# kidusabe1/Imagined-Speech-Decoding

Measured on AMD Instinct MI355X. Metric: trials/sec end-to-end (filterbank+CNN fwd+bwd), higher is better.
Workload: dtype f32; 1 GPU; cfg2: 64ch x 2s@256Hz EEG, 9-band Butterworth(4) filterbank -> STFT(64/32) log band power -> Conv4Layers(576,32)+Linear(32,5) fwd+bwd, softmax-CE, AdamW; trials_per_gpu=4096, global_batch=4096, parallelism=dp1, streams=one stream

## Files before the change

imagined-speech-decoding_amd/_lib.py:

```python
import ctypes as C
import os

from .build import LIB_PATH

ISD_OK = 0
ISD_ERR_INVALID, ISD_ERR_UNSUPPORTED, ISD_ERR_HIP, ISD_ERR_NO_DEVICE = -1, -2, -3, -4
FB_F32, FB_F64, FB_AUTO, FB_MIXED = 0, 1, 2, 3
BP_MAGNITUDE, BP_POWER, BP_LOGPOWER = 0, 1, 2


class IsdError(RuntimeError):
    def __init__(self, code, msg):
        super().__init__(f"libisd_hip error {code}: {msg}")
        self.code = code


class IsdUnsupported(IsdError):
    pass


_p, _i, _i64, _f = C.c_void_p, C.c_int, C.c_int64, C.c_float
_pi, _pd = C.POINTER(C.c_int), C.POINTER(C.c_double)

SIGNATURES = {
    "isd_abi_version": (_i, []),
    "isd_last_error": (C.c_char_p, []),
    "isd_shader_clock_probe": (_i, [_p, _i, _p]),
    "isd_wall_clock_khz": (_i, []),
    "isd_exact_sum_workspace_bytes": (_i64, []),
    "isd_exact_sum": (_i, [_p, _i64, _p, _p, _p]),
    "isd_device_count": (_i, []),
    "isd_adamw_step": (_i, [_p, _p, _p, _p, _i64, C.c_double, C.c_double, C.c_double, C.c_double, C.c_double, _i64,
                       _p, _p, _p]),
    "isd_adamw_multi_step": (_i, [_i, _p, _p, _p, _p, _p, C.c_double, C.c_double, C.c_double, C.c_double, C.c_double,
                             _i64, _p, _p, _p]),
    "isd_fb_plan_create": (_i, [C.POINTER(_p), _i, _i, _pd, _pd, _i]),
    "isd_fb_plan_destroy": (_i, [_p]),
    "isd_fb_plan_precision": (_i, [_p]),
    "isd_fb_forward": (_i, [_p, _p, _p, _i64, _i64, _i64, _p]),
    "isd_stft_plan_create": (_i, [C.POINTER(_p), _i, _i, _i]),
    "isd_stft_plan_destroy": (_i, [_p]),
    "isd_stft_plan_frames": (_i, [_p]),
    "isd_stft_plan_bins": (_i, [_p]),
    "isd_stft_forward": (_i, [_p, _p, _p, _i64, _p]),
    "isd_stft_bandpower": (_i, [_p, _p, _p, _i64, _i64, _i, _i, _pi, _pi, _i, _f, _p]),
    "isd_features_fused": (_i, [_p, _p, _p, _p, _i64, _i64, _pi, _pi, _i, _f, _p]),
    "isd_features_fused_bf16": (_i, [_p, _p, _p, _p, _i64, _i64, _pi, _pi, _i, _f, _p]),
    "isd_features_fused_last_path": (_i, []),
    "isd_features_backward_workspace_bytes": (_i64, [_p, _p, _i64, _i64, _pi, _pi]),
    "isd_features_backward": (_i, [_p, _p, _p, _p, _p, _p, _i64, _i64, _pi, _pi, _i, _f, _p]),
    "isd_attr_mix": (_i, [_p, _p, _p, _p, _p, _i64, _i64, _i, _i64, _i, _p]),
    "isd_attr_accumulate": (_i, [_p, _p, _p, _p, _p, _i64, _i64, _i, _i64, _i, _f, _p]),
    "isd_fir_plan_create": (_i, [C.POINTER(_p), _i, _pd]),
    "isd_fir_plan_destroy": (_i, [_p]),
    "isd_fir_plan_taps": (_i, [_p]),
    "isd_fir_zero_phase_f32": (_i, [_p, _p, _p, _i64, _i, _p]),
    "isd_fir_zero_phase_f64": (_i, [_p, _p, _p, _i64, _i, _p]),
    "isd_conv4_plan_create": (_i, [C.POINTER(_p), _i, _i, _pi, _pi, _i, _i, _i, _i]),
    "isd_conv4_plan_destroy": (_i, [_p]),
    "isd_conv4_plan_set_activation_dtype": (_i, [_p, _i]),
    "isd_conv4_param_count": (_i64, [_p]),
    "isd_conv4_param_offset": (_i64, [_p, _i, _i]),
    "isd_conv4_windows": (_i, [_p, _i64]),
    "isd_conv4_workspace_bytes": (_i64, [_p, _i64, _i64]),
    "isd_conv4_forward": (_i, [_p, _p, _p, _p, _p, _i64, _i64, _p]),
    "isd_conv4_backward": (_i, [_p, _p, _p, _p, _p, _p, _i64, _i64, _p]),
    "isd_conv4_backward_x": (_i, [_p, _p, _p, _p, _p, _p, _p, _i64, _i64, _p]),
    "isd_linear_forward": (_i, [_p, _p, _p, _p, _p, _i64, _i, _i, _i, _p]),
    "isd_linear_residual_forward": (_i, [_p, _p, _p, _p, _p, _i64, _i, _i, _p]),
    "isd_linear_workspace_bytes": (_i64, [_i64, _i, _i]),
    "isd_embed_forward": (_i, [_p, _p, _p, _p, _i64, _i, _i, _p]),
    "isd_embed_backward": (_i, [_p, _p, _p, _p, _i64, _i, _i, _p]),
    "isd_layernorm_forward": (_i, [_p, _p, _p, _p, _p, _i64, _i, _f, _p]),
    "isd_layernorm_backward": (_i, [_p, _p, _p, _p, _p, _p, _p, _i64, _i, _p]),
    "isd_attention_forward": (_i, [_p, _p, _p, _i64, _i, _i, _i, _f, C.c_uint64, _p]),
    "isd_attention_backward": (_i, [_p, _p, _p, _p, _i64, _i, _i, _i, _f, C.c_uint64, _p]),
    "isd_tail_fused_supported": (_i, [_i, _i, _i, _i, _i, _i]),
    "isd_tail_fused_param_count": (_i64, [_i, _i, _i, _i]),
    "isd_tail_fused_save_floats": (_i64, [_i64, _i, _i, _i]),
    "isd_tail_fused_workspace_floats": (_i64, [_i64, _i, _i, _i, _i, _i]),
    "isd_tail_fused_forward": (_i, [_p, _p, _p, _p, _p, _i64, _i, _i, _i, _i, _i, _i, _i, _f, _f, _f, C.c_uint64, _p,
                                    _p]),
    "isd_tail_fused_backward": (_i, [_p, _p, _p, _p, _p, _p, _p, _i64, _i, _i, _i, _i, _i, _i, _i, _f, _f, _f,
                                     C.c_uint64, _p, _p]),
    "isd_linear_backward": (_i, [_p, _p, _p, _p, _p, _p, _p, _p, _i64, _i, _i, _i, _p]),
    "isd_eegnet_plan_create": (_i, [C.POINTER(_p), _i, _i, _i, _i]),
    "isd_featcnn_supported": (_i, [_p, _i64, _i64, _i]),
    "isd_featcnn_step": (_i, [_p, _p, _p, _p, _p, _p, _i, _p, _p, _p, _p, _p, _p, _i64, _i64, _i, _f, _p]),
    "isd_featcnn_step_bf16": (_i, [_p, _p, _p, _p, _p, _p, _i, _p, _p, _p, _p, _p, _p, _i64, _i64, _i, _f, _p]),
    "isd_paperhead_plan_create": (_i, [C.POINTER(_p), _i, _i, _i]),
    "isd_paperhead_plan_destroy": (_i, [_p]),
    "isd_paperhead_param_count": (_i64, [_p]),
    "isd_paperhead_buffer_count": (_i64, [_p]),
    "isd_paperhead_workspace_bytes": (_i64, [_p, _i64]),
    "isd_paperhead_forward": (_i, [_p, _p, _p, _p, _p, _p, _i64, _i, _f, _f, _p]),
    "isd_paperhead_backward": (_i, [_p, _p, _p, _p, _p, _p, _i64, _p]),
    "isd_paperhead_backward_x": (_i, [_p, _p, _p, _p, _p, _p, _p, _i64, _i, _p]),
    "isd_paperhead_forward_stage": (_i, [_p, _i, _p, _p, _p, _p, _p, _i64, _i, _f, _f, _i, _p]),
    "isd_paperhead_backward_stage": (_i, [_p, _i, _p, _p, _p, _p, _p, _i64, _i, _p]),
    "isd_paperhead_sync_block": (_i, [_p, _i64, _i, _i, C.POINTER(C.c_int64), C.POINTER(C.c_int64)]),
    "isd_paperhead_sync_block_kind": (_i, [_i, _i]),
    "isd_eegnet_sync_block_kind": (_i, [_i, _i]),
    "isd_zone_batch_begin": (_i, []),
    "isd_zone_batch_next": (_i, []),
    "isd_zone_batch_launch": (_i, [_p]),
    "isd_zone_batch_abort": (_i, []),
    "isd_cvblock_plan_create": (_i, [C.POINTER(_p), _i, _i, _i]),
    "isd_cvblock_flat_dim": (_i64, [_p]),
    "isd_eegnet_plan_set_seed_counter": (_i, [_p, _p]),
    "isd_eegnet_plan_set_input_dtype": (_i, [_p, _i]),
    "isd_eegnet_plan_destroy": (_i, [_p]),
    "isd_eegnet_param_count": (_i64, [_p]),
    "isd_eegnet_buffer_count": (_i64, [_p]),
    "isd_eegnet_workspace_bytes": (_i64, [_p, _i64]),
    "isd_eegnet_forward": (_i, [_p, _p, _p, _p, _p, _p, _i64, _i, _f, _f, _f, C.c_uint64, _p]),
    "isd_eegnet_backward": (_i, [_p, _p, _p, _p, _p, _p, _i64, _f, C.c_uint64, _p]),
    "isd_eegnet_backward_x": (_i, [_p, _p, _p, _p, _p, _p, _p, _i64, _i, _f, C.c_uint64, _p]),
    "isd_eegnet_forward_stage": (_i, [_p, _i, _p, _p, _p, _p, _p, _i64, _i, _f, _f, _f, C.c_uint64, _i, _p]),
    "isd_eegnet_backward_stage": (_i, [_p, _i, _p, _p, _p, _p, _p, _i64, _f, C.c_uint64, _i, _p]),
    "isd_eegnet_sync_block": (_i, [_p, _i64, _i, _i, C.POINTER(_i64), C.POINTER(_i64)]),
    "isd_softmax_ce_workspace_bytes": (_i64, [_i64]),
    "isd_softmax_ce": (_i, [_p, _p, _i, _p, _p, _p, _p, _i64, _i, _i, _f, _p, _p]),
}

_lib = None


def lib():
    global _lib
    if _lib is None:
        if not os.path.exists(LIB_PATH):
# ... 28 lines not shown
```

imagined-speech-decoding_amd/csrc/fb.hip:

```cpp
#include "common.h"
#include "stft_plan.h"
#include <math.h>
#include <stdlib.h>
#include <vector>
#include <string.h>
#include <type_traits>
#include <atomic>

namespace isd {

constexpr int kL = 32;
constexpr int kSeg = 16 * kL;
constexpr int kPad = kL + 4;
constexpr int kMaxSec = 8;
constexpr int64_t kMaxRows = 0x7fffffffLL / (8 * 8);

struct FbSec {
  double Mp[4][4];
  double P[4];
  double N16d[4];
  double a1d, a2d;
  double hdq[2][kL / 2];
  float a1f, a2f;
  float N16f[4];
// ... 1132 lines not shown
              const float2 sv = rq[kk * 32 + sl];
              R[kk] += (f2){sv.x, sv.y};
            }
          }
        }
        const float2 wn = tw[(4 * j) & (nblk4 - 1)];
        float acc = 0.f;
#pragma unroll
        for (int bq = 0; bq < KB - 2; ++bq) {
          if (bq < nbin) {
            const f2 lo = R[bq], mid = R[bq + 1], hi = R[bq + 2];
            const float sx = hi.x * wn.x + hi.y * wn.y + lo.x * wn.x - lo.y * wn.y;
            const float sy = hi.y * wn.x - hi.x * wn.y + lo.y * wn.x + lo.x * wn.y;
            const float vx = 0.5f * mid.x + 0.25f * sx, vy = 0.5f * mid.y + 0.25f * sy;
            const float pw = (vx * vx + vy * vy) * scale2;
            acc += mode == ISD_BP_MAGNITUDE ? sqrtf(pw) : pw;
          }
        }
        float r = nbin > 0 ? acc / (float)nbin : 0.f;
        if (mode == ISD_BP_LOGPOWER) r = logf(r + eps);
        if (row_ok && j >= 0 && j < J) store_feat(out, j, r, out16);
      }
      wave_lds_sync();
    }
  }
}

__device__ __forceinline__ void ser_dma16(const void* src_lane, unsigned lds_base) {
  asm volatile("s_mov_b32 m0, %0\n\ts_nop 0\n\tglobal_load_lds_dwordx4 %1, off"
               :: "s"(__builtin_amdgcn_readfirstlane(lds_base)), "v"(src_lane) : "memory", "m0");
}

__device__ __forceinline__ float fma_to(float a, float b, float c) {
  float d;
  asm("v_fma_f32 %0, %1, %2, %3" : "=v"(d) : "s"(a), "v"(b), "v"(c));
  return d;
}
__device__ __forceinline__ void fma_over(double& d, double a, double b, double c) {
  asm("v_fma_f64 %0, %1, %2, %3" : "+v"(d) : "s"(a), "v"(b), "v"(c));
}
__device__ __forceinline__ void fma_over_mid(double& d, double a, double c) {
  asm("v_fma_f64 %0, %1, %0, %2" : "+v"(d) : "s"(a), "v"(c));
}

__device__ __forceinline__ void section_serial_f32(f2 (&v)[kL / 2], const SerSec& sc0, double& c1, double& c2) {
  const SerSec& sc = *later(&sc0);
  const float na1 = -sc.a1, na2 = -sc.a2;
  const float n16[4] = {sc.N16[0], sc.N16[1], sc.N16[2], sc.N16[3]};
  const double m0 = sc.M[0], m1 = sc.M[1], m2 = sc.M[2], m3 = sc.M[3];
  float h0[kL / 2], h1[kL / 2];
#pragma unroll
  for (int j = 0; j < kL / 2; ++j) { h0[j] = sc.hq[0][j]; h1[j] = sc.hq[1][j]; }
  const float one = sc.one;
  const f2 NA1 = {na1, na1}, NA2 = {na2, na2}, ONE = {one, one};
  f2 S1 = {0.f, 0.f}, S2 = {0.f, 0.f};
#pragma unroll
  for (int j = 0; j < kL / 2; ++j) {
    const f2 x = v[j];
    const f2 y = j == 0 ? x : __builtin_elementwise_fma(ONE, x, S1);
    S1 = j == 0 ? NA1 * y : __builtin_elementwise_fma(NA1, y, S2);
    S2 = __builtin_elementwise_fma(NA2, y, -x);
    v[j] = y;
  }
  const float sA1 = S1.x, sA2 = S2.x;
  const double e1 = (double)fmaf(n16[0], S1.x, fmaf(n16[1], S2.x, S1.y));
  const double e2 = (double)fmaf(n16[2], S1.x, fmaf(n16[3], S2.x, S2.y));
  const float t1 = (float)c1, t2 = (float)c2;
  const double i1 = fma(m1, c2, e1), i2 = fma(m3, c2, e2);
  fma_over(c2, m2, c1, i2);
  fma_over_mid(c1, m0, i1);
  const float u1 = fma_to(n16[0], t1, fmaf(n16[1], t2, sA1));
  const float u2 = fma_to(n16[2], t1, fmaf(n16[3], t2, sA2));
  const f2 T1 = {t1, u1}, T2 = {t2, u2};
#pragma unroll
  for (int j = 0; j < kL / 2; ++j)
    v[j] = __builtin_elementwise_fma((f2){h0[j], h0[j]}, T1, __builtin_elementwise_fma((f2){h1[j], h1[j]}, T2, v[j]));
}

constexpr int kSerRows = 64;
constexpr int kSerBins = 4;
constexpr int kSerMaxGroups = 4;

constexpr int kSerMaxWaves = 12;
template <int BPW, bool MAG>
__global__ __launch_bounds__(64 * kSerMaxWaves) __attribute__((amdgpu_waves_per_eu(BPW == 1 ? 5 : BPW == 2 ? 4 : 3)))
void fused_serial_kernel(const SerSec* __restrict__ secs, const FbBand* __restrict__ bands,
                         const float2* __restrict__ sym, const float* __restrict__ x, float* __restrict__ feat,
                         int R, int C, int T, int nb, int J, float scale2, FusedBands fbnd, int mode, float eps,
                         const int* __restrict__ bmap, int nb_out, int out16, int NW) {
  constexpr int NS = 4;
  extern __shared__ __attribute__((aligned(16))) float ring_raw[];
  const int lane = threadIdx.x & 63;
  const int wave_all = __builtin_amdgcn_readfirstlane((int)(threadIdx.x >> 6));
  const int grp = wave_all / NW, wave = wave_all - grp * NW;
  float* const ring = ring_raw + grp * (2 * kSerRows * kL);
  const int row0 = (blockIdx.x * (int)(blockDim.x >> 6) / NW + grp) * kSerRows;
  const int row = row0 + lane;
  const bool row_ok = row < R;
  const int rowc = row_ok ? row : R - 1;
  const int bt = rowc / C, ch = rowc - bt * C;
  unsigned obyte = (unsigned)(((int64_t)bt * nb_out * C + ch) * (int64_t)J) << (out16 ? 1 : 2);
  asm volatile("" : "+v"(obyte));
  const int64_t bstride = (int64_t)C * J;
  const int n_chunks = T / kL;

  const unsigned ring_base = (unsigned)(uintptr_t)(__attribute__((address_space(3))) float*)ring;
  auto fetch_tile = [&](int c) {
    if (c >= n_chunks) return;
    for (int i = wave; i < 8; i += NW) {
      const int r = 8 * i + (lane >> 3);
      int gr = row0 + r;
      gr = gr < R ? gr : R - 1;
      const float* src = x + (int64_t)gr * T + c * kL + 4 * ((lane & 7) ^ ((r >> 1) & 7));
      ser_dma16(src, ring_base + (unsigned)(((c & 1) * kSerRows * kL) * 4 + i * 1024));
    }
  };
  const int rbase = lane * kL, rswz = (lane >> 1) & 7;

  double S[BPW][NS][2];
  f2 prevU[BPW][kSerBins];
  float ob[BPW][4];
#pragma unroll
  for (int i = 0; i < BPW; ++i) {
    ob[i][0] = ob[i][1] = ob[i][2] = ob[i][3] = 0.f;
#pragma unroll
    for (int s = 0; s < NS; ++s) S[i][s][0] = S[i][s][1] = 0.0;
#pragma unroll
    for (int kk = 0; kk < kSerBins; ++kk) prevU[i][kk] = (f2){0.f, 0.f};
  }

  int pend = 0;
  fetch_tile(0);
  for (int c = 0; c <= n_chunks; ++c) {
    const bool last = c == n_chunks;
    const float* tile = ring + (c & 1) * (kSerRows * kL);
    if (pend == 1) __builtin_amdgcn_s_waitcnt(0x0F71);
    else if (pend == 2) __builtin_amdgcn_s_waitcnt(0x0F72);
    else if (pend == 3) __builtin_amdgcn_s_waitcnt(0x0F73);
    else __builtin_amdgcn_s_waitcnt(0x0F70);
    __builtin_amdgcn_s_barrier();
    asm volatile("" ::: "memory");
    fetch_tile(c + 1);
    pend = 0;
#pragma unroll
    for (int i = 0; i < BPW; ++i) {
      const int b = wave + i * NW;
      if (b < nb) {
        const int klo = fbnd.klo[b], khi = fbnd.khi[b];
        const int k0 = klo - 1, nbin = khi - klo + 1;
        f2 Xs[kSerBins];
        if (!last) {
          f2 v[kL / 2];
          {
            const float gain = bands[b].gf;
#pragma unroll
            for (int qd = 0; qd < 4; ++qd) {
              const float4 a = *reinterpret_cast<const float4*>(&tile[rbase + ((qd ^ rswz) << 2)]);
              const float4 h = *reinterpret_cast<const float4*>(&tile[rbase + (((qd + 4) ^ rswz) << 2)]);
#pragma unroll
              for (int e = 0; e < 4; ++e)
                v[4 * qd + e] = (f2){mul_unpacked(f4_get(a, e), gain), mul_unpacked(f4_get(h, e), gain)};
            }
          }
#pragma unroll
          for (int s = 0; s < NS; ++s) section_serial_f32(v, secs[b * NS + s], S[i][s][0], S[i][s][1]);
          f2 ad[15];
#pragma unroll
          for (int m = 1; m < 16; ++m) ad[m - 1] = sym_pair(v[m], v[16 - m]);
#pragma unroll
          for (int kk = 0; kk < kSerBins; ++kk) {
            const int k = k0 + kk;
            const f2* __restrict__ tq = later(reinterpret_cast<const f2*>(sym + (int64_t)k * 16));
            f2 tc[17];
#pragma unroll
            for (int m = 1; m <= 16; ++m) tc[m] = tq[m - 1];
            f2 acc_a = pmac0(ad[0], tc[1]), acc_b = pmac0(ad[1], tc[2]);
#pragma unroll
            for (int m = 3; m <= 13; m += 2) {
              pmac(acc_a, ad[m - 1], tc[m]);
              pmac(acc_b, ad[m], tc[m + 1]);
            }
            pmac(acc_a, ad[14], tc[15]);
            cmac_lo_conj(acc_b, v[0], tc[16]);
            f2 U = acc_a + acc_b;
            add_lo(U, v[0]);
            const float sg = __builtin_bit_cast(float, 0x3f800000u | ((unsigned)k << 31));
            Xs[kk] = __builtin_elementwise_fma(U, (f2){sg, sg}, prevU[i][kk]);
            prevU[i][kk] = U;
          }
        } else {
#pragma unroll
          for (int kk = 0; kk < kSerBins; ++kk) Xs[kk] = prevU[i][kk];
        }
        float acc = 0.f;
#pragma unroll
        for (int bq = 0; bq < kSerBins - 2; ++bq) {
          const f2 w = Xs[bq] - Xs[bq + 2], mid = Xs[bq + 1];
          const float vx = fmaf(0.25f, w.y, 0.5f * mid.x), vy = fmaf(-0.25f, w.x, 0.5f * mid.y);
          float pw = (vx * vx + vy * vy) * scale2;
          if (MAG) pw = sqrtf(pw);
          acc += bq < nbin ? pw : 0.f;
        }
        float r = acc * fbnd.inv[b];
        if (mode == ISD_BP_LOGPOWER) r = fast_log(r + eps);
        const int cq = c & 3;
        if (cq == 0) ob[i][0] = r; else if (cq == 1) ob[i][1] = r; else if (cq == 2) ob[i][2] = r; else ob[i][3] = r;
        if ((cq == 3 || last) && row0 < R) pend += (cq == 3) ? 1 : cq + 1;
        if (row_ok && (cq == 3 || last)) {
          const int64_t ou = (int64_t)bmap[b] * bstride + (c - cq);
          if (out16) {
            char* fu = reinterpret_cast<char*>(reinterpret_cast<unsigned short*>(feat) + ou) + obyte;
            if (cq == 3) {
              unsigned p0, p1;
              asm("v_cvt_pk_bf16_f32 %0, %1, %2" : "=v"(p0) : "v"(ob[i][0]), "v"(ob[i][1]));
              asm("v_cvt_pk_bf16_f32 %0, %1, %2" : "=v"(p1) : "v"(ob[i][2]), "v"(ob[i][3]));
              typedef unsigned u2h __attribute__((ext_vector_type(2), aligned(2)));
              *reinterpret_cast<u2h*>(fu) = (u2h){p0, p1};
            } else {
#pragma unroll
              for (int k = 0; k < 3; ++k)
                if (k <= cq) {
                  unsigned pk;
                  asm("v_cvt_pk_bf16_f32 %0, %1, %1" : "=v"(pk) : "v"(ob[i][k]));
                  reinterpret_cast<unsigned short*>(fu)[k] = (unsigned short)pk;
                }
            }
          } else {
            char* fu = reinterpret_cast<char*>(feat + ou) + obyte;
            if (cq == 3) {
              typedef float f4u __attribute__((ext_vector_type(4), aligned(4)));
              *reinterpret_cast<f4u*>(fu) = (f4u){ob[i][0], ob[i][1], ob[i][2], ob[i][3]};
            } else {
#pragma unroll
              for (int k = 0; k < 3; ++k)
                if (k <= cq) reinterpret_cast<float*>(fu)[k] = ob[i][k];
            }
          }
        }
      }
    }
  }
}

static void mat2_mul(const double* a, const double* b, double* o) {
  double r[4] = {a[0] * b[0] + a[1] * b[2], a[0] * b[1] + a[1] * b[3], a[2] * b[0] + a[3] * b[2],
                 a[2] * b[1] + a[3] * b[3]};
  memcpy(o, r, sizeof(r));
}

}

using namespace isd;

extern "C" int isd_fb_plan_destroy(isd_fb_plan* p);

static int rows4_share(int nb) {
  int best = kLongShare;
  double best_w = 1e30;
  for (int s = kLongShare; s >= 4; --s) {
    const int per = (nb + s - 1) / s;
    if (per > kRows4Bands) continue;
    const double w = (double)per * s / (double)(nb > 0 ? nb : 1);
    if (w < best_w - 1e-9) { best_w = w; best = s; }
  }
  return best;
}

static bool rows4_enabled() {
  static const bool on = getenv("ISD_FUSED_ROWS4_OFF") == nullptr;
  return on;
}

static bool rows4_reg_carry() {
  static const bool on = getenv("ISD_ROWS4_LDS_CARRY") == nullptr;
  return on;
}

static void build_section(double a1, double a2, FbSec& sc, double* Qout) {
  const double A[4] = {-a1, 1.0, -a2, 0.0};
  double An[4] = {1, 0, 0, 1};
  for (int k = 0; k < kL; ++k) {
    if (k < kL / 2) {
      sc.hdq[0][k] = An[0];
      sc.hdq[1][k] = An[1];
      sc.hq[0][k] = (float)An[0];
      sc.hq[1][k] = (float)An[1];
    }
    if (k == kL / 2)
      for (int e = 0; e < 4; ++e) {
        sc.N16d[e] = An[e];
        sc.N16f[e] = (float)An[e];
      }
    mat2_mul(A, An, An);
  }
  double Mk[4];
  memcpy(Mk, An, sizeof(Mk));
  double Qi[4] = {1, 0, 0, 1};
  for (int i = 0; i < 16; ++i) {
    memcpy(Qout + i * 4, Qi, sizeof(Qi));
    mat2_mul(Mk, Qi, Qi);
  }
  memcpy(sc.P, Qi, sizeof(Qi));
  for (int k = 0; k < 4; ++k) {
    memcpy(sc.Mp[k], Mk, sizeof(Mk));
    mat2_mul(Mk, Mk, Mk);
  }
  sc.a1d = a1; sc.a2d = a2; sc.a1f = (float)a1; sc.a2f = (float)a2;
}

extern "C" int isd_fb_plan_create(isd_fb_plan** out, int n_bands, int n_sections, const double* a12,
                                  const double* gain, int precision) {
  ISD_CHECK_ARG(out && a12 && gain, "isd_fb_plan_create: null argument");
  ISD_CHECK_ARG(n_bands >= 1 && n_bands <= 4096, "isd_fb_plan_create: n_bands=%d out of range", n_bands);
  ISD_CHECK_ARG(n_sections >= 1 && n_sections <= kMaxSec, "isd_fb_plan_create: n_sections=%d not in [1,%d]",
                n_sections, kMaxSec);
  ISD_CHECK_ARG(precision == ISD_FB_F32 || precision == ISD_FB_F64 || precision == ISD_FB_AUTO,
                "isd_fb_plan_create: bad precision %d", precision);
  const int n = n_bands * n_sections;
  std::vector<FbSec> secs(n);
  std::vector<FbBand> bands(n_bands);
  std::vector<double> Q((size_t)n * 64);
  std::vector<double> worst(n_bands, 0.0);
  for (int b = 0; b < n_bands; ++b) {
    bands[b].gd = gain[b];
// ... 92 lines not shown
    FbSet& fs = p->set[k];
    if (fs.d_sec) (void)hipFree(fs.d_sec);
    if (fs.d_band) (void)hipFree(fs.d_band);
    if (fs.d_Q) (void)hipFree(fs.d_Q);
    if (fs.d_map) (void)hipFree(fs.d_map);
    if (fs.d_ser) (void)hipFree(fs.d_ser);
    delete[] p->host_map[k];
  }
  delete p;
  return ISD_OK;
}

extern "C" int isd_fb_plan_precision(const isd_fb_plan* p) { return p ? p->precision : ISD_ERR_INVALID; }

template <typename VT, int GPR>
static int fb_launch(const isd_fb_plan* p, const FbSet& fs, const float* x, float* y, int64_t R, int C, int T,
                     hipStream_t st) {
  const int64_t items = cdiv(R, (int64_t)(4 / GPR));
  const int vec = ((T & 3) == 0) && ((reinterpret_cast<uintptr_t>(x) & 15) == 0) &&
                  ((reinterpret_cast<uintptr_t>(y) & 15) == 0);
  if (vec && T == GPR * kSeg && R % (4 / GPR) == 0)
    hipLaunchKernelGGL((fb_kernel<VT, GPR, true>), dim3((unsigned)items), dim3(64), 0, st, fs.d_sec, fs.d_band, fs.d_Q, x,
                       y, (int)R, C, T, fs.nb, p->n_sections, vec, fs.d_map, p->n_bands);
  else
    hipLaunchKernelGGL((fb_kernel<VT, GPR>), dim3((unsigned)items), dim3(64), 0, st, fs.d_sec, fs.d_band, fs.d_Q, x, y,
                       (int)R, C, T, fs.nb, p->n_sections, vec, fs.d_map, p->n_bands);
  ISD_LAUNCH_CHECK();
  return ISD_OK;
}

template <typename VT>
static int fb_launch_t(const isd_fb_plan* p, const FbSet& fs, const float* x, float* y, int64_t R, int C, int T,
                       hipStream_t st) {
  if (T <= kSeg) return fb_launch<VT, 1>(p, fs, x, y, R, C, T, st);
  if (T <= 2 * kSeg) return fb_launch<VT, 2>(p, fs, x, y, R, C, T, st);
  const int vec = ((T & 3) == 0) && ((reinterpret_cast<uintptr_t>(x) & 15) == 0) &&
                  ((reinterpret_cast<uintptr_t>(y) & 15) == 0);
  if (vec && T % kSeg == 0 && fs.nb <= kMaxBands && rows4_enabled()) {
    const int share_n = rows4_share(fs.nb);
    const dim3 grid4((unsigned)(cdiv(cdiv(R, 4), 8) * 8 * share_n));
#define ISD_R4(K) hipLaunchKernelGGL(K, grid4, dim3(64), 0, st, fs.d_sec, fs.d_band, fs.d_Q, x, y, C, T, fs.nb, \
                                     p->n_sections, fs.d_map, p->n_bands, (int)R, share_n)
    const bool fullq = R % 4 == 0;
    if (std::is_same<VT, float>::value) { if (fullq) ISD_R4(fb_rows4_kernel_f32<true>); else ISD_R4(fb_rows4_kernel_f32<false>); }
    else { if (fullq) ISD_R4(fb_rows4_kernel_f64<true>); else ISD_R4(fb_rows4_kernel_f64<false>); }
#undef ISD_R4
    ISD_LAUNCH_CHECK();
    return ISD_OK;
  }
  const dim3 grid((unsigned)(cdiv(R, 8) * 8 * kLongShare));
#define ISD_FBL(K) hipLaunchKernelGGL(K, grid, dim3(64), 0, st, fs.d_sec, fs.d_band, fs.d_Q, x, y, C, T, fs.nb, \
                                      p->n_sections, fs.d_map, p->n_bands, (int)R)
  if (std::is_same<VT, float>::value) { if (vec) ISD_FBL(fb_long_kernel_f32<true>); else ISD_FBL(fb_long_kernel_f32<false>); }
  else { if (vec) ISD_FBL(fb_long_kernel_f64<true>); else ISD_FBL(fb_long_kernel_f64<false>); }
#undef ISD_FBL
  ISD_LAUNCH_CHECK();
  return ISD_OK;
}

extern "C" int isd_fb_forward(const isd_fb_plan* p, const float* x, float* y, int64_t B, int64_t C, int64_t T,
                              void* stream) {
  ISD_CHECK_ARG(p, "isd_fb_forward: null plan");
  ISD_CHECK_ARG(B >= 0 && C >= 1 && T >= 1 && T <= (1 << 24) && C <= (1 << 20), "isd_fb_forward: bad shape B=%lld C=%lld T=%lld",
                (long long)B, (long long)C, (long long)T);
  if (B == 0) return ISD_OK;
  ISD_CHECK_ARG(x && y, "isd_fb_forward: null argument");
  hipStream_t st = (hipStream_t)stream;
  const int64_t R = B * C;
  ISD_CHECK_ARG(R <= kMaxRows, "isd_fb_forward: too many rows (%lld)", (long long)R);
  int rc = ISD_OK;
  if (p->set[0].nb) rc = fb_launch_t<float>(p, p->set[0], x, y, R, (int)C, (int)T, st);
  if (rc == ISD_OK && p->set[1].nb) rc = fb_launch_t<double>(p, p->set[1], x, y, R, (int)C, (int)T, st);
  return rc;
}

static void set_band(FusedBands& f, int i, int klo, int khi) {
  f.klo[i] = klo;
  f.khi[i] = khi;
  f.inv[i] = khi >= klo ? 1.f / (float)(khi - klo + 1) : 0.f;
}

static thread_local int g_fused_path = 0;
extern "C" int isd_features_fused_last_path(void) { return g_fused_path; }

static bool serial_wanted() {
  const char* e = getenv("ISD_FUSED_SERIAL");
  return !(e && e[0] == '0');
}

static void serial_lds_limit() {
  static std::atomic<unsigned long long> done{0};
  int dev = 0;
  if (hipGetDevice(&dev) != hipSuccess || dev < 0 || dev >= 64) dev = 0;
  const unsigned long long bit = 1ull << dev;
  if (done.load(std::memory_order_relaxed) & bit) return;
  const int lds = (int)(sizeof(float) * kSerMaxGroups * 2 * kSerRows * kL);
  const void* k[] = {(const void*)fused_serial_kernel<1, false>, (const void*)fused_serial_kernel<1, true>,
                     (const void*)fused_serial_kernel<2, false>, (const void*)fused_serial_kernel<2, true>,
                     (const void*)fused_serial_kernel<3, false>, (const void*)fused_serial_kernel<3, true>};
  for (const void* f : k) (void)hipFuncSetAttribute(f, hipFuncAttributeMaxDynamicSharedMemorySize, lds);
  done.fetch_or(bit, std::memory_order_relaxed);
}

static bool fused_serial_launch(const isd_fb_plan* fb, const FbSet& fs, const isd_stft_plan* st, const float* x,
                                float* feat, int64_t R, int C, const FusedBands& fbnd, int mode, float eps,
                                hipStream_t stream, int out16) {
  if (!serial_wanted() || !st->d_sym || !fs.d_ser || st->n != 64 || st->hop != 32 || st->T % kL != 0 || st->T < kL) return false;
  if (st->J != st->T / kL + 1 || fb->n_sections != 4 || (reinterpret_cast<uintptr_t>(x) & 15) != 0) return false;
  if (fs.nb < 1 || fs.nb > 12) return false;
  if (cdiv(R, C) * (int64_t)fb->n_bands * C * st->J * 4 >= (1LL << 31)) return false;
  for (int i = 0; i < fs.nb; ++i) {
    const int nbin = fbnd.khi[i] - fbnd.klo[i] + 1;
    if (nbin < 1 || nbin > kSerBins - 2 || fbnd.klo[i] < 1 || fbnd.khi[i] > st->n / 2 - 1) return false;
  }
  int bpw = 3;
  if (const char* e = getenv("ISD_SERIAL_BPW")) { const int v = atoi(e); if (v >= 1 && v <= 3) bpw = v; }
  while (bpw < 3 && (fs.nb + bpw - 1) / bpw > kSerMaxWaves) ++bpw;
  const int nw = (fs.nb + bpw - 1) / bpw;
  bpw = (fs.nb + nw - 1) / nw;
  int groups = nw % 4 == 0 ? 1 : nw % 2 == 0 ? 2 : 4;
  while (groups > 1 && groups * nw > kSerMaxWaves) groups >>= 1;
  if (const char* e = getenv("ISD_SERIAL_GROUPS")) { const int v = atoi(e); if (v >= 1 && v <= kSerMaxGroups && v * nw <= kSerMaxWaves) groups = v; }
  const dim3 grid((unsigned)cdiv(R, (int64_t)kSerRows * groups));
  const size_t lds = sizeof(float) * (size_t)groups * 2 * kSerRows * kL;
  const bool mag = mode == ISD_BP_MAGNITUDE;
  if (lds > 48 * 1024) serial_lds_limit();
#define ISD_SER(BPW_)                                                                                                   \
  do {                                                                                                                  \
    if (mag)                                                                                                            \
      hipLaunchKernelGGL((fused_serial_kernel<BPW_, true>), grid, dim3(64 * nw * groups), lds, stream, fs.d_ser,        \
                         fs.d_band, st->d_sym, x, feat, (int)R, C, st->T, fs.nb, st->J, st->scale * st->scale, fbnd,    \
                         mode, eps, fs.d_map, fb->n_bands, out16, nw);                                                  \
    else                                                                                                                \
      hipLaunchKernelGGL((fused_serial_kernel<BPW_, false>), grid, dim3(64 * nw * groups), lds, stream, fs.d_ser,       \
                         fs.d_band, st->d_sym, x, feat, (int)R, C, st->T, fs.nb, st->J, st->scale * st->scale, fbnd,    \
                         mode, eps, fs.d_map, fb->n_bands, out16, nw);                                                  \
  } while (0)
  if (bpw == 1) ISD_SER(1);
  else if (bpw == 2) ISD_SER(2);
  else ISD_SER(3);
#undef ISD_SER
  return true;
}

template <typename VT>
static int fused_launch(const isd_fb_plan* fb, const FbSet& fs, const isd_stft_plan* st, const float* x, float* feat,
                        int64_t R, int C, const FusedBands& fbnd, int mode, float eps, hipStream_t stream, int out16) {
  if (std::is_same<VT, float>::value &&
      fused_serial_launch(fb, fs, st, x, feat, R, C, fbnd, mode, eps, stream, out16)) {
    g_fused_path = 2;
    ISD_LAUNCH_CHECK();
    return ISD_OK;
  }
  if (std::is_same<VT, float>::value) g_fused_path = 1;
  const bool two = st->T > kSeg;
  const int64_t items = cdiv(R, two ? 2 : 4);
  const int vec = ((st->T & 3) == 0) && ((reinterpret_cast<uintptr_t>(x) & 15) == 0);
  const int gpr = two ? 2 : 1;
  const bool full = vec && st->T == gpr * kSeg && R % (4 / gpr) == 0;
#define ISD_FUSED3(M, G, F)                                                                                          \
  hipLaunchKernelGGL((fused_kernel<VT, M, G, F>), dim3((unsigned)items), dim3(64), 0, stream, fs.d_sec, fs.d_band,   \
                     fs.d_Q, st->d_dft, x, feat, (int)R, C, st->T, fs.nb, fb->n_sections, st->J,                     \
                     st->scale * st->scale, fbnd, mode, eps, vec, fs.d_map, fb->n_bands, out16)
#define ISD_FUSED(M, G) do { if (full) ISD_FUSED3(M, G, true); else ISD_FUSED3(M, G, false); } while (0)
  if (mode == ISD_BP_MAGNITUDE) { if (two) ISD_FUSED(true, 2); else ISD_FUSED(true, 1); }
  else { if (two) ISD_FUSED(false, 2); else ISD_FUSED(false, 1); }
#undef ISD_FUSED3
#undef ISD_FUSED
  ISD_LAUNCH_CHECK();
  return ISD_OK;
}

static int features_fused_impl(const isd_fb_plan* fb, const isd_stft_plan* st, const float* x, float* feat,
                               int64_t B, int64_t C, const int* klo, const int* khi, int mode, float eps,
                               void* stream, int out16) {
  ISD_CHECK_ARG(fb && st, "isd_features_fused: null plan");
  ISD_CHECK_ARG(B == 0 || (x && feat), "isd_features_fused: null argument");
  ISD_CHECK_ARG(B >= 0 && C >= 1 && C <= (1 << 20), "isd_features_fused: bad shape B=%lld C=%lld", (long long)B,
                (long long)C);
  ISD_CHECK_ARG(mode >= ISD_BP_MAGNITUDE && mode <= ISD_BP_LOGPOWER, "isd_features_fused: bad mode %d", mode);
  const bool short_rows = st->n == 64 && st->hop == 32 && st->T <= 2 * kSeg && st->d_dft;
  const bool long_rows = st->d_blk && st->hop == 64 && st->T <= 64 * 64;
  if (!short_rows && !long_rows) {
    set_error("isd_features_fused: needs nperseg=64/noverlap=32/T<=1024, or hop 64 with nperseg = 2^a*64 and T<=4096 "
              "(got nperseg=%d hop=%d T=%d)", st->n, st->hop, st->T);
    return ISD_ERR_UNSUPPORTED;
  }
  FusedBands all = {};
  int rc = fill_band_args(st, fb->n_bands, klo, khi, all.klo, all.khi, "isd_features_fused");
  if (rc) return rc;
  if (B == 0) return ISD_OK;
  ISD_CHECK_ARG(B * C <= kMaxRows, "isd_features_fused: too many rows (%lld)", (long long)(B * C));
  hipStream_t s = (hipStream_t)stream;
  if (!short_rows) {
    g_fused_path = 3;
    int nbmax = 0;
    for (int b = 0; b < fb->n_bands; ++b) {
      const int nbin = all.khi[b] - all.klo[b] + 1;
      if (nbin < 1 || nbin > 6 || all.klo[b] < 1 || all.khi[b] > st->n / 2 - 1) {
        set_error("isd_features_fused: band %d needs 1..6 interior bins for the block-sum path (bins %d..%d)", b,
                  all.klo[b], all.khi[b]);
        return ISD_ERR_UNSUPPORTED;
      }
      if (nbin > nbmax) nbmax = nbin;
    }
    const int64_t rows = B * C;
    int log2_nblk = 0;
    while ((64 << log2_nblk) < st->n) ++log2_nblk;
    const int KB = nbmax + 2 <= 4 ? 4 : nbmax + 2 <= 5 ? 5 : nbmax + 2 <= 6 ? 6 : 8;
    const int n_iter = (st->T + 4 * kSeg - 1) / (4 * kSeg);
    const int vec = ((st->T & 3) == 0) && ((reinterpret_cast<uintptr_t>(x) & 15) == 0);
    for (int k = 0; k < 2; ++k) {
      const FbSet& fs = fb->set[k];
      if (!fs.nb) continue;
      FusedBands fbnd = {};
      for (int i = 0; i < fs.nb; ++i) set_band(fbnd, i, all.klo[fb->host_map[k][i]], all.khi[fb->host_map[k][i]]);
      const size_t lds = sizeof(float2) * ((size_t)KB * 64 + 64) + sizeof(double) * (2 * kMaxSec + 64 * kMaxSec);
#define ISD_FL_LAUNCH2(VT, K, V)                                                                                      \
  hipLaunchKernelGGL((fused_long_kernel<VT, K, V>), dim3((unsigned)(cdiv(rows, 8) * 8 * kLongShare)), dim3(64), lds, s, \
                     fs.d_sec, fs.d_band, fs.d_Q, st->d_blk, x, feat, (int)C, st->T, fs.nb, fb->n_sections, st->J,      \
                     log2_nblk, st->n / 2, st->scale * st->scale, fbnd, mode, eps, fs.d_map, fb->n_bands, (int)rows, \
                     out16)
      const bool rows4 = vec && st->T % kSeg == 0 && log2_nblk <= 4 && log2_nblk >= 1 && rows4_enabled();
// ... 355 lines not shown
```

include/isd_hip.h:

```cpp
#ifndef ISD_HIP_H
#define ISD_HIP_H

#include <stdint.h>

#ifdef __cplusplus
extern "C" {
#endif

#define ISD_ABI_VERSION 1

enum {
  ISD_OK = 0,
  ISD_ERR_INVALID = -1,
  ISD_ERR_UNSUPPORTED = -2,
  ISD_ERR_HIP = -3,
  ISD_ERR_NO_DEVICE = -4
};

int isd_abi_version(void);
const char* isd_last_error(void);
int isd_shader_clock_probe(uint64_t* out, int spin_us, void* stream);
int isd_wall_clock_khz(void);
int64_t isd_exact_sum_workspace_bytes(void);
int isd_exact_sum(const float* x, int64_t n, double* out, void* workspace, void* stream);
int isd_device_count(void);

typedef struct isd_fb_plan isd_fb_plan;

enum { ISD_FB_F32 = 0, ISD_FB_F64 = 1, ISD_FB_AUTO = 2, ISD_FB_MIXED = 3  };

int isd_fb_plan_create(isd_fb_plan** out, int n_bands, int n_sections,
                       const double* a12, const double* gain, int precision);
int isd_fb_plan_destroy(isd_fb_plan* plan);
int isd_fb_plan_precision(const isd_fb_plan* plan);

int isd_fb_forward(const isd_fb_plan* plan, const float* x, float* y,
                   int64_t B, int64_t C, int64_t T, void* stream);

typedef struct isd_stft_plan isd_stft_plan;

int isd_stft_plan_create(isd_stft_plan** out, int T, int nperseg, int noverlap);
int isd_stft_plan_destroy(isd_stft_plan* plan);
int isd_stft_plan_frames(const isd_stft_plan* plan);
int isd_stft_plan_bins(const isd_stft_plan* plan);

int isd_stft_forward(const isd_stft_plan* plan, const float* x, float* Z,
                     int64_t R, void* stream);

enum {
  ISD_BP_MAGNITUDE = 0,
  ISD_BP_POWER = 1,
  ISD_BP_LOGPOWER = 2
};

int isd_stft_bandpower(const isd_stft_plan* plan, const float* y, float* feat,
                       int64_t B, int64_t C, int n_bands_in, int n_bands,
                       const int* klo, const int* khi, int mode, float eps, void* stream);

int isd_features_fused(const isd_fb_plan* fb, const isd_stft_plan* st, const float* x,
                       float* feat, int64_t B, int64_t C, const int* klo, const int* khi,
                       int mode, float eps, void* stream);
int isd_features_fused_bf16(const isd_fb_plan* fb, const isd_stft_plan* st, const float* x, uint16_t* feat,
                            int64_t B, int64_t C, const int* klo, const int* khi, int mode, float eps, void* stream);

int isd_features_fused_last_path(void);

int64_t isd_features_backward_workspace_bytes(const isd_fb_plan* fb, const isd_stft_plan* st, int64_t B, int64_t C,
                                              const int* klo, const int* khi);
int isd_features_backward(const isd_fb_plan* fb, const isd_stft_plan* st, const float* x, const float* dfeat,
                          float* dx, void* workspace, int64_t B, int64_t C, const int* klo, const int* khi,
                          int mode, float eps, void* stream);

int isd_attr_mix(const float* x, const float* bg, const int32_t* ridx, const float* alpha, float* out,
                 int64_t n_pairs, int64_t pair0, int S, int64_t E, int M, void* stream);
int isd_attr_accumulate(const float* x, const float* bg, const int32_t* ridx, const float* grad, float* acc,
                        int64_t n_pairs, int64_t pair0, int S, int64_t E, int M, float scale, void* stream);

typedef struct isd_fir_plan isd_fir_plan;
int isd_fir_plan_create(isd_fir_plan** out, int n_taps, const double* taps);
int isd_fir_plan_destroy(isd_fir_plan* plan);
int isd_fir_plan_taps(const isd_fir_plan* plan);
int isd_fir_zero_phase_f32(const isd_fir_plan* plan, const float* x, float* y, int64_t rows, int T, void* stream);
int isd_fir_zero_phase_f64(const isd_fir_plan* plan, const double* x, double* y, int64_t rows, int T, void* stream);

typedef struct isd_conv4_plan isd_conv4_plan;

int isd_conv4_plan_create(isd_conv4_plan** out, int c_total, int n_zones, const int* zone_sizes,
                          const int* zone_channels, int feature_dim, int n_layers, int window_len,
                          int slide_step);
int isd_conv4_plan_destroy(isd_conv4_plan* plan);
enum { ISD_ACT_F32 = 0, ISD_ACT_BF16 = 1 };
int isd_conv4_plan_set_activation_dtype(isd_conv4_plan* plan, int dtype);
int64_t isd_conv4_param_count(const isd_conv4_plan* plan);
int64_t isd_conv4_param_offset(const isd_conv4_plan* plan, int zone, int which);
int isd_conv4_windows(const isd_conv4_plan* plan, int64_t T);
int64_t isd_conv4_workspace_bytes(const isd_conv4_plan* plan, int64_t B, int64_t T);

int isd_conv4_forward(const isd_conv4_plan* plan, const float* x, const float* params, float* feat,
                      void* workspace, int64_t B, int64_t T, void* stream);
int isd_conv4_backward(const isd_conv4_plan* plan, const float* x, const float* params,
                       const float* dfeat, float* dparams, void* workspace, int64_t B, int64_t T,
                       void* stream);
int isd_conv4_backward_x(const isd_conv4_plan* plan, const float* x, const float* params, const float* dfeat,
                         float* dparams, float* dx, void* workspace, int64_t B, int64_t T, void* stream);

int isd_linear_forward(const float* x, const float* w, const float* bias, float* y, float* pre,
                       int64_t M, int K, int N, int act, void* stream);
int isd_linear_residual_forward(const float* x, const float* w, const float* bias, const float* res, float* y,
                                int64_t M, int K, int N, void* stream);
int64_t isd_linear_workspace_bytes(int64_t M, int K, int N);
int isd_linear_backward(const float* x, const float* w, const float* dy, const float* pre, float* dx,
                        float* dw, float* db, void* workspace, int64_t M, int K, int N, int act,
                        void* stream);

int64_t isd_softmax_ce_workspace_bytes(int64_t B);
int isd_softmax_ce(const float* logits_tok, const void* labels, int label_bytes, float* logits_mean,
                   float* loss, float* dlogits_tok, int64_t* pred, int64_t B, int n_tok, int n_cls,
                   float grad_scale, void* workspace, void* stream);

typedef struct isd_eegnet_plan isd_eegnet_plan;
int isd_eegnet_plan_create(isd_eegnet_plan** out, int in_channels, int feature_dim, int kernel_length, int T);
int isd_cvblock_plan_create(isd_eegnet_plan** out, int in_channels, int dim_token, int T);
int64_t isd_cvblock_flat_dim(const isd_eegnet_plan* plan);
int isd_eegnet_plan_set_seed_counter(isd_eegnet_plan* plan, const uint64_t* seed_dev);
int isd_eegnet_plan_set_input_dtype(isd_eegnet_plan* plan, int dtype);
int isd_eegnet_plan_destroy(isd_eegnet_plan* plan);
int64_t isd_eegnet_param_count(const isd_eegnet_plan* plan);
int64_t isd_eegnet_buffer_count(const isd_eegnet_plan* plan);
int64_t isd_eegnet_workspace_bytes(const isd_eegnet_plan* plan, int64_t B);
int isd_eegnet_forward(const isd_eegnet_plan* plan, const float* x, const float* params, float* buffers,
                       float* out, void* workspace, int64_t B, int training, float momentum, float eps,
                       float dropout_p, uint64_t seed, void* stream);
int isd_eegnet_backward(const isd_eegnet_plan* plan, const float* x, const float* params, const float* dout,
                        float* dparams, void* workspace, int64_t B, float dropout_p, uint64_t seed,
                        void* stream);
int isd_eegnet_backward_x(const isd_eegnet_plan* plan, const float* x, const float* params, const float* dout,
                          float* dparams, float* dx, void* workspace, int64_t B, int training, float dropout_p,
                          uint64_t seed, void* stream);
int isd_eegnet_forward_stage(const isd_eegnet_plan* plan, int stage, const float* x, const float* params,
                             float* buffers, float* out, void* workspace, int64_t B, int training, float momentum,
                             float eps, float dropout_p, uint64_t seed, int world, void* stream);
int isd_eegnet_backward_stage(const isd_eegnet_plan* plan, int stage, const float* x, const float* params,
                              const float* dout, float* dparams, void* workspace, int64_t B, float dropout_p,
                              uint64_t seed, int world, void* stream);
int isd_eegnet_sync_block(const isd_eegnet_plan* plan, int64_t B, int backward, int stage, int64_t* byte_offset,
                          int64_t* n_doubles);
int isd_eegnet_sync_block_kind(int backward, int stage);

// ... 74 lines not shown
```

Before: 3.809 million trials/s.

## Stage fused-serial filterbank features in LDS and flush coalesced per frame piece

Adds a staged variant of the fused serial filterbank+STFT kernel. It writes per-row band-power outputs into an LDS staging buffer and flushes them in frame chunks, with lanes spread across rows and frames, instead of each lane scattering 4-frame groups directly to global memory. It also raises the dynamic LDS limit to the full CU size so a staging buffer fits, and sizes the chunk from the occupancy budget. The cost is extra LDS use, which may reduce occupancy, plus extra wave syncs around the flushes.

After: 3.801 million trials/s. No clear change (-0.2%).

```diff
diff --git a/imagined-speech-decoding_amd/_lib.py b/imagined-speech-decoding_amd/_lib.py
--- a/imagined-speech-decoding_amd/_lib.py
+++ b/imagined-speech-decoding_amd/_lib.py
@@ -47,6 +47,7 @@
     "isd_features_fused": (_i, [_p, _p, _p, _p, _i64, _i64, _pi, _pi, _i, _f, _p]),
     "isd_features_fused_bf16": (_i, [_p, _p, _p, _p, _i64, _i64, _pi, _pi, _i, _f, _p]),
     "isd_features_fused_last_path": (_i, []),
+    "isd_features_fused_last_stage": (_i, []),
     "isd_features_backward_workspace_bytes": (_i64, [_p, _p, _i64, _i64, _pi, _pi]),
     "isd_features_backward": (_i, [_p, _p, _p, _p, _p, _p, _i64, _i64, _pi, _pi, _i, _f, _p]),
     "isd_attr_mix": (_i, [_p, _p, _p, _p, _p, _i64, _i64, _i, _i64, _i, _p]),
diff --git a/imagined-speech-decoding_amd/csrc/fb.hip b/imagined-speech-decoding_amd/csrc/fb.hip
--- a/imagined-speech-decoding_amd/csrc/fb.hip
+++ b/imagined-speech-decoding_amd/csrc/fb.hip
@@ -1238,12 +1238,12 @@
 constexpr int kSerMaxGroups = 4;
 
 constexpr int kSerMaxWaves = 12;
-template <int BPW, bool MAG>
+template <int BPW, bool MAG, bool STG>
 __global__ __launch_bounds__(64 * kSerMaxWaves) __attribute__((amdgpu_waves_per_eu(BPW == 1 ? 5 : BPW == 2 ? 4 : 3)))
 void fused_serial_kernel(const SerSec* __restrict__ secs, const FbBand* __restrict__ bands,
                          const float2* __restrict__ sym, const float* __restrict__ x, float* __restrict__ feat,
                          int R, int C, int T, int nb, int J, float scale2, FusedBands fbnd, int mode, float eps,
-                         const int* __restrict__ bmap, int nb_out, int out16, int NW) {
+                         const int* __restrict__ bmap, int nb_out, int out16, int NW, int FS) {
   constexpr int NS = 4;
   extern __shared__ __attribute__((aligned(16))) float ring_raw[];
   const int lane = threadIdx.x & 63;
@@ -1273,6 +1273,55 @@
   };
   const int rbase = lane * kL, rswz = (lane >> 1) & 7;
 
+  const int SS = FS | 1;
+  const int n_pieces = STG ? (J + FS - 1) / FS : 1;
+  float* const stg = ring_raw + (int)(blockDim.x >> 6) / NW * (2 * kSerRows * kL) + wave_all * (BPW * kSerRows * SS + kSerRows);
+  unsigned* const otab = reinterpret_cast<unsigned*>(stg + BPW * kSerRows * SS);
+  float* const stg_lane = stg + lane * SS;
+  if (STG) otab[lane] = row_ok ? obyte : ~0u;
+  auto flush = [&](int f0, int L) {
+    wave_lds_sync();
+    const int q = kSerRows / L, rm = kSerRows - q * L;
+    const int fr0 = lane / L, ff0 = lane - fr0 * L;
+#pragma unroll
+    for (int i = 0; i < BPW; ++i) {
+      const int b = wave + i * NW;
+      if (b < nb) {
+        const int64_t ou = (int64_t)bmap[b] * bstride + f0;
+        char* const fu = out16 ? reinterpret_cast<char*>(reinterpret_cast<unsigned short*>(feat) + ou)
+                               : reinterpret_cast<char*>(feat + ou);
+        int fr = fr0, ff = ff0;
+        for (int k0 = 0; k0 < L; k0 += 4) {
+          float rv[4];
+          unsigned ro[4], fo[4];
+#pragma unroll
+          for (int u = 0; u < 4; ++u) {
+            const int frc = fr < kSerRows ? fr : kSerRows - 1;
+            rv[u] = stg[(i * kSerRows + frc) * SS + ff];
+            ro[u] = otab[frc];
+            fo[u] = (unsigned)ff;
+            fr += q; ff += rm;
+            if (ff >= L) { ff -= L; ++fr; }
+          }
+#pragma unroll
+          for (int u = 0; u < 4; ++u) {
+            if (k0 + u < L && ro[u] != ~0u) {
+              if (out16) {
+                unsigned pk;
+                asm("v_cvt_pk_bf16_f32 %0, %1, %1" : "=v"(pk) : "v"(rv[u]));
+                *reinterpret_cast<unsigned short*>(fu + (ro[u] + 2u * fo[u])) = (unsigned short)pk;
+              } else {
+                *reinterpret_cast<float*>(fu + (ro[u] + 4u * fo[u])) = rv[u];
+              }
+            }
+          }
+        }
+      }
+    }
+  };
+  int pc_lo = 0, pc_hi = J / n_pieces, pc_i = 0;
+  int fl_lo = 0, fl_n = 0;
+
   double S[BPW][NS][2];
   f2 prevU[BPW][kSerBins];
   float ob[BPW][4];
@@ -1296,6 +1345,7 @@
     else __builtin_amdgcn_s_waitcnt(0x0F70);
     __builtin_amdgcn_s_barrier();
     asm volatile("" ::: "memory");
+    if (STG && fl_n) { flush(fl_lo, fl_n); fl_n = 0; }
     fetch_tile(c + 1);
     pend = 0;
 #pragma unroll
@@ -1359,6 +1409,10 @@
         }
         float r = acc * fbnd.inv[b];
         if (mode == ISD_BP_LOGPOWER) r = fast_log(r + eps);
+        if (STG) {
+          stg_lane[i * kSerRows * SS + (c - pc_lo)] = r;
+          continue;
+        }
         const int cq = c & 3;
         if (cq == 0) ob[i][0] = r; else if (cq == 1) ob[i][1] = r; else if (cq == 2) ob[i][2] = r; else ob[i][3] = r;
         if ((cq == 3 || last) && row0 < R) pend += (cq == 3) ? 1 : cq + 1;
@@ -1395,7 +1449,13 @@
         }
       }
     }
-  }
+    if (STG && c + 1 == pc_hi) {
+      fl_lo = pc_lo; fl_n = pc_hi - pc_lo;
+      pc_lo = pc_hi; ++pc_i;
+      pc_hi = (pc_i + 1) * J / n_pieces;
+    }
+  }
+  if (STG && fl_n) flush(fl_lo, fl_n);
 }
 
 static void mat2_mul(const double* a, const double* b, double* o) {
@@ -1654,24 +1714,53 @@
 
 static thread_local int g_fused_path = 0;
 extern "C" int isd_features_fused_last_path(void) { return g_fused_path; }
+static thread_local int g_fused_stage = 0;
+extern "C" int isd_features_fused_last_stage(void) { return g_fused_stage; }
 
 static bool serial_wanted() {
   const char* e = getenv("ISD_FUSED_SERIAL");
   return !(e && e[0] == '0');
 }
 
-static void serial_lds_limit() {
-  static std::atomic<unsigned long long> done{0};
+constexpr int kSerLdsCU = 160 * 1024;
+static int serial_lds_limit() {
+  static std::atomic<unsigned long long> done{0}, wide{0};
   int dev = 0;
   if (hipGetDevice(&dev) != hipSuccess || dev < 0 || dev >= 64) dev = 0;
   const unsigned long long bit = 1ull << dev;
-  if (done.load(std::memory_order_relaxed) & bit) return;
-  const int lds = (int)(sizeof(float) * kSerMaxGroups * 2 * kSerRows * kL);
-  const void* k[] = {(const void*)fused_serial_kernel<1, false>, (const void*)fused_serial_kernel<1, true>,
-                     (const void*)fused_serial_kernel<2, false>, (const void*)fused_serial_kernel<2, true>,
-                     (const void*)fused_serial_kernel<3, false>, (const void*)fused_serial_kernel<3, true>};
-  for (const void* f : k) (void)hipFuncSetAttribute(f, hipFuncAttributeMaxDynamicSharedMemorySize, lds);
-  done.fetch_or(bit, std::memory_order_relaxed);
+  const int tiles = (int)(sizeof(float) * kSerMaxGroups * 2 * kSerRows * kL);
+  if (done.load(std::memory_order_acquire) & bit) return (wide.load(std::memory_order_relaxed) & bit) ? kSerLdsCU : tiles;
+#define ISD_SER_K(B_) (const void*)fused_serial_kernel<B_, false, false>, (const void*)fused_serial_kernel<B_, true, false>, \
+                      (const void*)fused_serial_kernel<B_, false, true>, (const void*)fused_serial_kernel<B_, true, true>
+  const void* k[] = {ISD_SER_K(1), ISD_SER_K(2), ISD_SER_K(3)};
+#undef ISD_SER_K
+  bool ok = true;
+  for (const void* f : k) ok = hipFuncSetAttribute(f, hipFuncAttributeMaxDynamicSharedMemorySize, kSerLdsCU) == hipSuccess && ok;
+  if (!ok) {
+    (void)hipGetLastError();
+    for (const void* f : k) (void)hipFuncSetAttribute(f, hipFuncAttributeMaxDynamicSharedMemorySize, tiles);
+  } else {
+    wide.fetch_or(bit, std::memory_order_relaxed);
+  }
+  done.fetch_or(bit, std::memory_order_release);
+  return ok ? kSerLdsCU : tiles;
+}
+
+static int serial_stage_frames(int J, int bpw, int waves, size_t tile_bytes, int lds_limit) {
+  const char* e = getenv("ISD_SERIAL_STAGE");
+  const int forced = e ? atoi(e) : -1;
+  if (forced == 0) return 0;
+  const int cap = bpw == 1 ? 5 : bpw == 2 ? 4 : 3;
+  const int resident = std::max(1, cap / ((waves + 3) / 4));
+  const int64_t budget = std::min<int64_t>(kSerLdsCU / resident / 2048 * 2048, lds_limit) - (int64_t)tile_bytes;
+  const int64_t ss_max = (budget / waves / 4 - kSerRows) / (bpw * kSerRows);
+  if (budget <= 0 || ss_max < 1) return 0;
+  int fs = (int)std::min<int64_t>(J, ss_max % 2 ? ss_max : ss_max - 1);
+  if (forced > 0) fs = std::min(fs, forced);
+  if (fs < 1) return 0;
+  if (fs < J && fs < 4 && forced <= 0) return 0;
+  const int pieces = (J + fs - 1) / fs;
+  return (J + pieces - 1) / pieces;
 }
 
 static bool fused_serial_launch(const isd_fb_plan* fb, const FbSet& fs, const isd_stft_plan* st, const float* x,
@@ -1694,23 +1783,24 @@
   while (groups > 1 && groups * nw > kSerMaxWaves) groups >>= 1;
   if (const char* e = getenv("ISD_SERIAL_GROUPS")) { const int v = atoi(e); if (v >= 1 && v <= kSerMaxGroups && v * nw <= kSerMaxWaves) groups = v; }
   const dim3 grid((unsigned)cdiv(R, (int64_t)kSerRows * groups));
-  const size_t lds = sizeof(float) * (size_t)groups * 2 * kSerRows * kL;
+  const size_t tiles = sizeof(float) * (size_t)groups * 2 * kSerRows * kL;
   const bool mag = mode == ISD_BP_MAGNITUDE;
-  if (lds > 48 * 1024) serial_lds_limit();
+  const int stage = serial_stage_frames(st->J, bpw, nw * groups, tiles, serial_lds_limit());
+  g_fused_stage = stage;
+  const size_t lds = tiles + (stage ? sizeof(float) * (size_t)(nw * groups) * (bpw * kSerRows * (stage | 1) + kSerRows) : 0);
+#define ISD_SER3(BPW_, MAG_, STG_)                                                                                     \
+  hipLaunchKernelGGL((fused_serial_kernel<BPW_, MAG_, STG_>), grid, dim3(64 * nw * groups), lds, stream, fs.d_ser,     \
+                     fs.d_band, st->d_sym, x, feat, (int)R, C, st->T, fs.nb, st->J, st->scale * st->scale, fbnd, mode,  \
+                     eps, fs.d_map, fb->n_bands, out16, nw, stage)
 #define ISD_SER(BPW_)                                                                                                   \
   do {                                                                                                                  \
-    if (mag)                                                                                                            \
-      hipLaunchKernelGGL((fused_serial_kernel<BPW_, true>), grid, dim3(64 * nw * groups), lds, stream, fs.d_ser,        \
-                         fs.d_band, st->d_sym, x, feat, (int)R, C, st->T, fs.nb, st->J, st->scale * st->scale, fbnd,    \
-                         mode, eps, fs.d_map, fb->n_bands, out16, nw);                                                  \
-    else                                                                                                                \
-      hipLaunchKernelGGL((fused_serial_kernel<BPW_, false>), grid, dim3(64 * nw * groups), lds, stream, fs.d_ser,       \
-                         fs.d_band, st->d_sym, x, feat, (int)R, C, st->T, fs.nb, st->J, st->scale * st->scale, fbnd,    \
-                         mode, eps, fs.d_map, fb->n_bands, out16, nw);                                                  \
+    if (mag) { if (stage) ISD_SER3(BPW_, true, true); else ISD_SER3(BPW_, true, false); }                               \
+    else { if (stage) ISD_SER3(BPW_, false, true); else ISD_SER3(BPW_, false, false); }                                 \
   } while (0)
   if (bpw == 1) ISD_SER(1);
   else if (bpw == 2) ISD_SER(2);
   else ISD_SER(3);
+#undef ISD_SER3
 #undef ISD_SER
   return true;
 }
diff --git a/include/isd_hip.h b/include/isd_hip.h
--- a/include/isd_hip.h
+++ b/include/isd_hip.h
@@ -64,6 +64,8 @@
                             int64_t B, int64_t C, const int* klo, const int* khi, int mode, float eps, void* stream);
 
 int isd_features_fused_last_path(void);
+
+int isd_features_fused_last_stage(void);
 
 int64_t isd_features_backward_workspace_bytes(const isd_fb_plan* fb, const isd_stft_plan* st, int64_t B, int64_t C,
                                               const int* klo, const int* khi);
```
